# neobotix/neo_mpc_planner2

Measured on AMD Instinct MI355X. Metric: MPC solves/sec (control_steps=3, 500x500 costmap), higher is better.
Workload: dtype f64

## Files before the change

neo_mpc_planner2_amd/csrc/adjoint.h:

```cpp
#pragma once
#include "neo_mpc_device.h"
#include "wave_ops.h"
#include "fast_math.h"
#include "solver_context.h"
#include "costmap.h"
#include "riccati.h"

namespace neo_mpc {
namespace {

template <bool kTame, bool kRiccati, int kFew = 0>
__device__ __forceinline__ void adjoint_by_scans(const SolveArgs& a, const Ctx& c, double* L, bool exact_step, int lane, int n,
                                                 bool& free_path, int& nhops) {
  auto scan = [](double v) { if constexpr (kFew > 0) return wave_scan_few<kFew>(v); else return wave_scan(v); };
  constexpr int kLast = kFew > 0 ? kFew - 1 : 63;
  const DevParams& p = a.p;
  const double* u = L + a.lds.u;
  double* gs = L + a.lds.gs;
  float* RS = reinterpret_cast<float*>(L + a.lds.ric);
  float* ARTF = reinterpret_cast<float*>(L + a.lds.rt);
  const bool on = lane < n;
  const double vx = on ? u[3 * lane] : 0.0, vy = on ? u[3 * lane + 1] : 0.0, w = on ? u[3 * lane + 2] : 0.0;
  const double th = scan(w * p.dt);
  double sn, cs;
  sincos_heading<kTame>(th, &sn, &cs);
  const double ddx = (vx * cs - vy * sn) * p.dt, ddy = (vx * sn + vy * cs) * p.dt;
  const double x = scan(ddx), y = scan(ddy);
  double rt = on ? -2.0 * p.wo_n * (c.tyaw - th) : 0.0;
  if (lane == n - 1) rt += -2.0 * p.wterm_o * (c.fyaw - th);
  const double rx = on ? -2.0 * p.wt_n * (c.cx - x) : 0.0, ry = on ? -2.0 * p.wt_n * (c.cy - y) : 0.0;
  const double px = scan(rx), py = scan(ry);
  const double SX = lane_value(px, kLast) - px + rx, SY = lane_value(py, kLast) - py + ry;
  const double tt = on ? rt - ddy * SX + ddx * SY : 0.0;
  const double pt = scan(tt);
  const double ST = lane_value(pt, kLast) - pt + tt;
  int raw_here = 0;
  bool has_hop = false;
  float hop_x = 0.0f, hop_y = 0.0f;
  if (on) {
    gs[3 * lane] = p.dt * (cs * SX + sn * SY);
    gs[3 * lane + 1] = p.dt * (-sn * SX + cs * SY);
    gs[3 * lane + 2] = p.dt * ST;
    if (kRiccati) {
      float* rs = RS + kRicStage * lane;
      rs[RS_CS] = (float)cs; rs[RS_SN] = (float)sn; rs[RS_PX] = (float)ddx; rs[RS_PY] = (float)ddy;
      double wxx, wxy, wyy, wlx, wly;
      raw_here = edge_stickiness(a, c, L, x, y, cs, sn, wxx, wxy, wyy, wlx, wly, has_hop, hop_x, hop_y);
      rs[RS_WXX] = (float)wxx; rs[RS_WXY] = (float)wxy; rs[RS_WYY] = (float)wyy;
      rs[RS_WLX] = (float)wlx; rs[RS_WLY] = (float)wly;
      rs[RS_SY] = exact_step ? (float)SY : 0.0f;
      ARTF[2 * lane + 1] = exact_step ? (float)SX : 0.0f;
    }
  }
  if (kRiccati) {
    free_path = __ballot(raw_here != 0) == 0ull;
    const unsigned long long hmask = __ballot(has_hop);
    const int rank = __popcll(hmask & ((1ull << lane) - 1ull));
    double* t = L + a.lds.tol;
    if (has_hop && rank < kHopLanes) {
      reinterpret_cast<int*>(t + T_HOP_STAGE)[rank] = lane;
      reinterpret_cast<float*>(t + T_HOP_VEC)[2 * rank] = hop_x;
      reinterpret_cast<float*>(t + T_HOP_VEC)[2 * rank + 1] = hop_y;
    }
    nhops = min(__popcll(hmask), (int)kHopLanes);
    if (lane == 0) reinterpret_cast<int*>(t + T_HOP_STAGE)[kHopLanes] = nhops;
  }
  WAVE_SYNC();
}

template <int kSteps, bool kTame>
__device__ __forceinline__ void adjoint_short_sweep(const SolveArgs& a, const Ctx& c, double* L, bool have_trig, int lane, int n) {
  const DevParams& p = a.p;
  const double* u = L + a.lds.u;
  double* gs = L + a.lds.gs;
  double* ACS = L + a.lds.cs;
  double* ASN = L + a.lds.sn;
  double* ADX = L + a.lds.dxs;
  double* ADY = L + a.lds.dys;
  double* ARX = L + a.lds.rx;
  double* ARY = L + a.lds.ry;
  double* ART = L + a.lds.rt;
  double x = 0.0, y = 0.0, th = 0.0;
#pragma unroll
  for (int i = 0; i < n; ++i) {
    const double vx = u[3 * i], vy = u[3 * i + 1], w = u[3 * i + 2];
    th += w * p.dt;
    double sn, cs;
    if (kSteps && have_trig) { sn = ASN[i]; cs = ACS[i]; }
    else sincos_heading<kTame>(th, &sn, &cs);
    const double ddx = (vx * cs - vy * sn) * p.dt, ddy = (vx * sn + vy * cs) * p.dt;
    x += ddx; y += ddy;
    double rt = -2.0 * p.wo_n * (c.tyaw - th);
    if (i == n - 1) rt += -2.0 * p.wterm_o * (c.fyaw - th);
    if (lane == 0) {
      ACS[i] = cs; ASN[i] = sn; ADX[i] = ddx; ADY[i] = ddy;
      ARX[i] = -2.0 * p.wt_n * (c.cx - x); ARY[i] = -2.0 * p.wt_n * (c.cy - y); ART[i] = rt;
    }
  }
  WAVE_SYNC();
  double SX = 0.0, SY = 0.0, ST = 0.0;
#pragma unroll
  for (int k = n - 1; k >= 0; --k) {
    SX += ARX[k]; SY += ARY[k];
    ST += ART[k] - ADY[k] * SX + ADX[k] * SY;
    if (lane == 0) {
      gs[3 * k] = p.dt * (ACS[k] * SX + ASN[k] * SY);
      gs[3 * k + 1] = p.dt * (-ASN[k] * SX + ACS[k] * SY);
      gs[3 * k + 2] = p.dt * ST;
    }
  }
  WAVE_SYNC();
}

}
}
```

neo_mpc_planner2_amd/csrc/costmap.h:

```cpp
#pragma once
#include <hip/hip_runtime.h>
#include <math.h>
#include <stdint.h>

#include "neo_mpc_device.h"
#include "wave_ops.h"
#include "solver_context.h"
#include "fast_math.h"
#include "solver_rules.h"

namespace neo_mpc {
namespace {

__device__ __forceinline__ int cell_of(double w, double origin, double res, double inv) {
  double t = w - origin;
  double q = t * inv;
  double fl = floor(q);
  if (fabs(q - rint(q)) < 1e-6) fl = floor(t / res);
  int cell;
  asm("v_cvt_i32_f64 %0, %1" : "=v"(cell) : "v"(fl));
  return cell;
}

__device__ __forceinline__ int map_raw(const DevMap& m, int mx, int my) {
  if (mx < -m.border || my < -m.border || mx >= m.size_x + m.border || my >= m.size_y + m.border)
    return 254;
  return m.cells[(long)my * m.pitch + mx];
}

__device__ __forceinline__ int raw_occupancy(int raw) {
  return raw == 0 ? 0 : raw == 253 ? 99 : raw == 254 ? 100 : raw == 255 ? -1 : 1 + (97 * (raw - 1)) / 251;
}
__device__ __forceinline__ double raw_cost(int raw) { return (double)raw_occupancy(raw) / 100.0; }

template <bool kCovered = false>
__device__ __forceinline__ int cell_raw(const SolveArgs& a, const Ctx& c, const double* L, int mx, int my) {
  const unsigned tx = (unsigned)(mx - c.tile_x0), ty = (unsigned)(my - c.tile_y0);
  const int lg = c.tile_geom & 31;
  if (kCovered || ((tx >> lg) == 0u && ty < (unsigned)(c.tile_geom >> 8)))
    return reinterpret_cast<const uint8_t*>(L + a.lds.tile)[(ty << lg) + tx];
  return map_raw(a.map, mx, my);
}

template <bool kCovered = false>
__device__ __forceinline__ int step_raw(const SolveArgs& a, const Ctx& c, const double* L, double x, double y) {
  if (c.tile_geom & kTileFree) return 0;
  const double X = c.X0 + (c.c0 * x - c.s0 * y), Y = c.Y0 + (c.s0 * x + c.c0 * y);
  const int mx = cell_of(X, a.map.origin_x, a.map.resolution, a.map.inv_resolution);
  const int my = cell_of(Y, a.map.origin_y, a.map.resolution, a.map.inv_resolution);
  return cell_raw<kCovered>(a, c, L, mx, my);
}
template <bool kCovered = false>
__device__ __forceinline__ double step_term(const SolveArgs& a, const Ctx& c, const double* L, double x, double y) {
  return L[a.lds.term + step_raw<kCovered>(a, c, L, x, y)];
}

constexpr double kSticky = NEO_RULE_STICKY, kWall = NEO_RULE_WALL, kStickyDist = NEO_RULE_STICKY_DIST, kWallDist = NEO_RULE_WALL_DIST;
constexpr double kHopMargin = NEO_RULE_HOP_MARGIN;
template <bool kCovered = false>
__device__ __forceinline__ int edge_stickiness(const SolveArgs& a, const Ctx& c, const double* L, double x, double y,
                                               double cs, double sn, double& wxx, double& wxy, double& wyy, double& lx,
                                               double& ly, bool& hop, float& hop_x, float& hop_y) {
  wxx = 0.0; wxy = 0.0; wyy = 0.0; lx = 0.0; ly = 0.0;
  hop = false; hop_x = 0.0f; hop_y = 0.0f;
  if (c.tile_geom & kTileFree) return 0;
  double wt_n = a.p.wt_n;
  asm volatile("" : "+s"(wt_n));
  const double X = c.X0 + (c.c0 * x - c.s0 * y), Y = c.Y0 + (c.s0 * x + c.c0 * y);
  const int mx = cell_of(X, a.map.origin_x, a.map.resolution, a.map.inv_resolution);
  const int my = cell_of(Y, a.map.origin_y, a.map.resolution, a.map.inv_resolution);
  const double fx = (X - a.map.origin_x) * a.map.inv_resolution - (double)mx;
  const double fy = (Y - a.map.origin_y) * a.map.inv_resolution - (double)my;
  const int raw_here = cell_raw<kCovered>(a, c, L, mx, my);
  const double here = L[a.lds.term + raw_here];
  const bool far = mx <= -2147483647 || mx >= 2147483646 || my <= -2147483647 || my >= 2147483646;
  if (far) return raw_here;
  const double hop_range = L[a.lds.tol + T_HOP_RANGE];
  const double zone = fmax(kWallDist, hop_range);
  const bool xlo = fx < zone, xhi = 1.0 - fx < zone, ylo = fy < zone, yhi = 1.0 - fy < zone;
  double rx = 0.0, ry = 0.0, pbx = 0.0, pby = 0.0;
  double drop = L[a.lds.tol + T_HOP_DROP], hwx = 0.0, hwy = 0.0;
  if (xlo || xhi) {
    const int raw_n = cell_raw<kCovered>(a, c, L, xlo ? mx - 1 : mx + 1, my);
    const double dist = xlo ? fx : 1.0 - fx, there = L[a.lds.term + raw_n];
    const bool wall = raw_n == 254 && raw_here != 254;
    if (wall) { if (dist < kWallDist) { rx = kWall * 2.0 * wt_n; pbx = (xlo ? kWallDist - dist : dist - kWallDist) * a.map.resolution; } }
    else if (dist < kStickyDist && there > here) rx = kSticky * 2.0 * wt_n;
    if (dist < hop_range && here - there > drop) {
      drop = here - there; hop = true;
      hwx = (xlo ? -1.0 : 1.0) * (dist + kHopMargin) * a.map.resolution; hwy = 0.0;
    }
  }
  if (ylo || yhi) {
    const int raw_n = cell_raw<kCovered>(a, c, L, mx, ylo ? my - 1 : my + 1);
    const double dist = ylo ? fy : 1.0 - fy, there = L[a.lds.term + raw_n];
    const bool wall = raw_n == 254 && raw_here != 254;
    if (wall) { if (dist < kWallDist) { ry = kWall * 2.0 * wt_n; pby = (ylo ? kWallDist - dist : dist - kWallDist) * a.map.resolution; } }
    else if (dist < kStickyDist && there > here) ry = kSticky * 2.0 * wt_n;
    if (dist < hop_range && here - there > drop) {
      hop = true;
      hwx = 0.0; hwy = (ylo ? -1.0 : 1.0) * (dist + kHopMargin) * a.map.resolution;
    }
  }
  wxx = rx * c.c0 * c.c0 + ry * c.s0 * c.s0;
  wxy = rx * c.c0 * -c.s0 + ry * c.s0 * c.c0;
  wyy = rx * c.s0 * c.s0 + ry * c.c0 * c.c0;
  lx = -(rx * pbx * c.c0 + ry * pby * c.s0);
  ly = -(rx * pbx * -c.s0 + ry * pby * c.c0);
  if (hop) {
    const double hrx = c.c0 * hwx + c.s0 * hwy, hry = -c.s0 * hwx + c.c0 * hwy, idt = rcp_fast(a.p.dt);
    hop_x = (float)((cs * hrx + sn * hry) * idt); hop_y = (float)((-sn * hrx + cs * hry) * idt);
  }
  return raw_here;
}

__device__ double edge_cost(const DevMap& m, double ax, double ay, double bx, double by) {
  int x0 = cell_of(ax, m.origin_x, m.resolution, m.inv_resolution);
  int y0 = cell_of(ay, m.origin_y, m.resolution, m.inv_resolution);
  const int x1 = cell_of(bx, m.origin_x, m.resolution, m.inv_resolution);
  const int y1 = cell_of(by, m.origin_y, m.resolution, m.inv_resolution);
  if (x0 < 0 || y0 < 0 || x0 >= m.size_x || y0 >= m.size_y || x1 < 0 || y1 < 0 || x1 >= m.size_x || y1 >= m.size_y)
    return raw_cost(254);
  const long dx = labs((long)x1 - x0), dy = labs((long)y1 - y0);
  const int sx = x1 >= x0 ? 1 : -1, sy = y1 >= y0 ? 1 : -1;
  long err = dx - dy;
  double worst = -1.0;
  for (long guard = 0; guard <= dx + dy + 1; ++guard) {
    worst = fmax(worst, raw_cost(map_raw(m, x0, y0)));
    if (x0 == x1 && y0 == y1) break;
    long e2 = 2 * err;
    if (e2 > -dy) { err -= dy; x0 += sx; }
    if (e2 < dx) { err += dx; y0 += sy; }
  }
  return worst;
}

__device__ double footprint_cost(const SolveArgs& a, const double* L, uint32_t b, int lane) {
  if (!a.footprints || a.footprint_points == 0) return L[a.lds.prob + P_FOOTPRINT];
  const int np = (int)a.footprint_points;
  const double* pts = a.footprints + (size_t)b * 2 * np;
  double worst = -1.0;
  for (int e = lane; e < np; e += kLanes) {
    int j = (e + 1) % np;
    worst = fmax(worst, edge_cost(a.map, pts[2 * e], pts[2 * e + 1], pts[2 * j], pts[2 * j + 1]));
  }
  return wave_max(worst);
}

}
}
```

neo_mpc_planner2_amd/csrc/k1_solve.h:

```cpp
#pragma once
#include <hip/hip_runtime.h>
#include <hip/hip_ext.h>
#include <math.h>
#include <stdint.h>
#include <stdlib.h>

#include "neo_mpc_device.h"
#include "wave_ops.h"
#include "fast_math.h"
#include "solver_context.h"
#include "solver_rules.h"
#include "costmap.h"
#include "feasible_set.h"
#include "rollout.h"
#include "riccati.h"
#include "adjoint.h"
#include "tangent_cone.h"
#include "dense_newton.h"
#include "lbfgs.h"
#include "cell_scan.h"
#include "k1_timing.h"

namespace neo_mpc {
namespace {
// ... 75 lines not shown
    select_map(a.map, L + a.lds.prob);
    flags = reset_and_warm(a, L, b, lane) ? NEO_MPC_FLAG_RESET : 0;
    const double fcost = footprint_cost(a, L, b, lane);
    if (lane == 0) L[a.lds.prob + P_FOOTPRINT] = fcost;
    Ctx c;
    make_ctx_wave(p, a.map, L + a.lds.prob, fcost, c, lane);
    load_tile(a, c, L, lane);
    s.wall_in_reach = (c.tile_geom & kTileWall) != 0;
    if (s.wall_in_reach) flags |= NEO_MPC_FLAG_WALL_IN_REACH;
    if (lane == 0) {
      double* t = L + a.lds.tol;
      t[T_XTOL] = p.xtol; t[T_EARLY] = p.early_tol; t[T_FINAL] = p.final_tol; t[T_FTOL] = p.ftol;
      t[T_STALL] = p.stall_step; t[T_WTOL] = p.wtol; t[T_WTOL_LATE] = p.wtol_late; t[T_KINK] = p.kink_radius;
      t[T_KONST] = c.konst; t[T_TRUE_YAW] = c.true_yaw;
      t[T_HOP_DROP] = p.hop_min_drop; t[T_HOP_RANGE] = p.hop_range;
      t[T_BTOL_MAP] = p.btol_map; t[T_BTOL_FREE] = p.btol_free;
      reinterpret_cast<int*>(t + T_HOP_STAGE)[kHopLanes] = 0;
      t[T_C0] = c.c0; t[T_S0] = c.s0; t[T_TYAW] = c.tyaw; t[T_FYAW] = c.fyaw;
      int* ti = reinterpret_cast<int*>(t + T_TILE);
      ti[0] = c.tile_x0; ti[1] = c.tile_y0; ti[2] = c.tile_geom;
    }
    double* u = L + a.lds.u;
    for (int i = lane; i < n; i += kLanes) project_block<kTame>(p, u[3 * i], u[3 * i + 1], u[3 * i + 2]);
    WAVE_SYNC();
    for (int k = 0; k < nv; ++k) cold = cold && (u[k] == 0.0);
    ctx_from_lds<false>(a, L, c);
    {
      double* S = L + a.lds.state;
      int* Si = reinterpret_cast<int*>(S);
      const bool has_prev = uniform_int(Si[SI_HAS_PREV]) == 1 && !(flags & NEO_MPC_FLAG_RESET);
      WAVE_SYNC();
      if (lane == 0) {
        double q0 = has_prev ? S[S_PREV_U0] : u[nv - 3], q1 = has_prev ? S[S_PREV_U0 + 1] : u[nv - 2], q2 = has_prev ? S[S_PREV_U0 + 2] : u[nv - 1];
        project_block<kTame>(p, q0, q1, q2);
        S[S_PREV_U0] = q0; S[S_PREV_U0 + 1] = q1; S[S_PREV_U0 + 2] = q2;
        Si[SI_HAS_PREV] = 0;
      }
      WAVE_SYNC();
    }
    if (!cold && n > 1 && !(p.compat & kCompatNoUnshift) && p.max_it < kDumpGradient) {
      const double* A0 = L + a.lds.state + S_PREV_U0;
      double ts = 0.0;
      const double fs = rollout_cost<kSteps, kTame, kCovered>(
          a, c, L,
          [&](int i, double& b0, double& b1, double& b2) {
            const double* src = lane == 1 ? (i == 0 ? A0 : u + 3 * (i - 1)) : u + 3 * i;
            b0 = src[0]; b1 = src[1]; b2 = src[2];
          },
          NoRecord(), &ts);
      const double f_warm = lane_value(fs, 0), f_alt = lane_value(fs, 1);
      const bool free_both = lane_value(ts, 0) == 0.0 && lane_value(ts, 1) == 0.0;
      if (f_alt < f_warm && free_both) {
        double v0 = 0.0, v1 = 0.0, v2 = 0.0;
        const int k0 = lane, k1 = lane + kLanes, k2 = lane + 2 * kLanes;
        if (k0 < nv) v0 = k0 >= 3 ? u[k0 - 3] : A0[k0];
        if (k1 < nv) v1 = u[k1 - 3];
        if (k2 < nv) v2 = u[k2 - 3];
        WAVE_SYNC();
        if (k0 < nv) u[k0] = v0;
        if (k1 < nv) u[k1] = v1;
        if (k2 < nv) u[k2] = v2;
      } else if (f_alt < f_warm && lane == 0) {
        reinterpret_cast<int*>(L + a.lds.state)[SI_HAS_PREV] = kAltArmed;
      }
      WAVE_SYNC();
    }
  }
  s.flags = flags; s.cold = cold;
  return true;
}

template <int kMinWavesPerSimd, int kSteps, int kDir, bool kTame, int kStaticTile, int kLayoutSteps, bool kRouted = false>
__device__ __forceinline__ bool solve_search(double* L, uint32_t b, SolveCarry& sc) {
  constexpr bool kCovered = kStaticTile > 0;
  constexpr bool kNewton = kDir == 1;
  constexpr bool kRiccati = kDir == 2;
  constexpr bool kSecond = kDir != 0;
  constexpr bool kBlockedRule = kNewton || kRouted;
  static_assert(!kRiccati || kSteps == 0 || kRouted, "the stage-wise direction: run-time-sized, or the routed kernel's control_steps-3 branch");
  static_assert(!kRouted || (kRiccati && kSteps == kRoutedSteps), "the routed branch is the stage-wise one, three stages in registers");
  constexpr int kFew = (kRiccati && kSteps > 0) ? kSteps : 0;
  constexpr bool kHandOff = kFew > 0;
  constexpr bool kScalarCase = kFew > 0 && kTame;
  constexpr int kNwSteps = !kNewton ? 1 : kSteps ? kSteps : kNewtonMaxSteps;
  constexpr bool kVectorPose = kTame;
  constexpr int kRegSteps = kSteps ? kSteps : 1;
  constexpr int kPairs = kSteps ? 4 : NEO_MPC_MAX_LBFGS_MEMORY;
  double f = sc.f;
  const bool cold = sc.cold;
  int npairs = 0, head = 0, nfev = sc.nfev, it = sc.it, status = sc.status;
  neo_search_run run;
  neo_search_run_init(&run);
  double u_term = 0.0;
  double alpha = 1.0;
  bool scanned = false;
  int nscans = 0;
  bool scan_only = false;
  auto lane_again = []() {
    int zero;
    asm volatile("v_mov_b32 %0, 0" : "=v"(zero));
    return (int)__builtin_amdgcn_mbcnt_hi(~0u, __builtin_amdgcn_mbcnt_lo(~0u, (unsigned)zero));
  };
  NEO_SEGMENT_DECL;
  NEO_SEGMENT(0);
  for (;;) {
  SolveArgs a;
  fresh_args<kSteps, kStaticTile, kLayoutSteps, kRouted>(a);
  own_loop_params(a);
  select_map(a.map, L + a.lds.prob);
  const DevParams& p = a.p;
  const int n = kSteps ? kSteps : p.n, nv = 3 * n, mem = p.mem;
  double cand[3 * kRegSteps], cand_sn[kRegSteps], cand_cs[kRegSteps];
  bool have_trig = false;
  Ctx c;
  ctx_from_lds<kVectorPose>(a, L, c);
  double* u = L + a.lds.u;
  double* gs = L + a.lds.gs;
  double* gt = L + a.lds.gt;
  double* gr = L + a.lds.gr;
  double* d = L + a.lds.d;
  double* u_prev = L + a.lds.u_prev;
  double* gt_prev = L + a.lds.gt_prev;
  double* u_new = L + a.lds.u_new;
  double* ACS = L + a.lds.cs;
  double* ASN = L + a.lds.sn;
  int* AMODE = reinterpret_cast<int*>(L + a.lds.mode);
  static_assert(2 * 7 >= kNewtonRecord, "Newton records do not fit the step arrays");

  if (!scanned && nscans == 0) {
    const int lane = lane_again();
    for (int i = lane; i < n; i += kLanes) { AMODE[4 * i + 2] = 0; AMODE[4 * i + 3] = 0; }
    if (kRouted && lane == 0) L[a.lds.tol + T_KINK] = p.kink_radius_stagewise;
    alpha = kRiccati ? fmax(1.0, n * 0.125) : 1.0;
    if (kFew && lane == 0) { double* t = L + a.lds.tol; t[T_GAIN1] = INFINITY; t[T_GAIN2] = INFINITY; t[T_ALPHA] = alpha; }
    if (kRiccati && lane == 0) L[a.lds.tol + T_MU] = n > 8 ? (double)(n - 8) * 0.125 : 0.0;
  }
  bool v_feasible = false;
  if (kRiccati) {
    double b0 = c.v0, b1 = c.v1, b2 = c.v2;
    asm volatile("" : "+v"(b0), "+v"(b1), "+v"(b2));
    project_block<kTame>(p, b0, b1, b2);
    v_feasible = b0 == c.v0 && b1 == c.v1 && b2 == c.v2;
  }
  double my_scale;
  {
    int l0 = lane_again();
    my_scale = kRiccati ? 0.0 : lane_scale<kSecond>(l0);
  }
  for (; it < p.max_it && !scan_only; ++it) {
    int lane = lane_again();
    const bool exact_step = kRiccati && run.nblocked == 0;
    int tol_off = a.lds.tol;
    asm volatile("" : "+s"(tol_off));
    const double* TOL = L + tol_off;
    NEO_PHASE_DECL;
    NEO_PHASE(0);
    constexpr int kVars = 3 * kNwSteps;
    const int nvr = kSteps ? kVars : nv;
    bool free_path = false;
    int nhops = 0;
    float hc[kVars];
    float newton_sol = 0.0f;
    float dm_reg = 0.0f;
    int near_reg = 0;
    if (kNewton) {
      double hcol[kSteps ? kVars : 1];
      const double hstep = 1e-6, inv_h = 1.0 / hstep;
      double pcs[kNwSteps], psn[kNwSteps];
      double x = 0.0, y = 0.0, th = 0.0;
    #pragma unroll
      for (int i = 0; i < kNwSteps; ++i) {
        if (kSteps || i < n) {
          const double vx = u[3 * i] + (lane == 3 * i ? hstep : 0.0);
          const double vy = u[3 * i + 1] + (lane == 3 * i + 1 ? hstep : 0.0);
          const double w = u[3 * i + 2] + (lane == 3 * i + 2 ? hstep : 0.0);
          th += w * p.dt;
          sincos_heading<kTame>(th, &psn[i], &pcs[i]);
          x += (vx * pcs[i] - vy * psn[i]) * p.dt;
          y += (vx * psn[i] + vy * pcs[i]) * p.dt;
        }
      }
      double SX = 0.0, SY = 0.0, ST = 0.0;
    #pragma unroll
      for (int k = kNwSteps - 1; k >= 0; --k) {
        if (kSteps || k < n) {
          const double vx = u[3 * k] + (lane == 3 * k ? hstep : 0.0);
          const double vy = u[3 * k + 1] + (lane == 3 * k + 1 ? hstep : 0.0);
          const double w = u[3 * k + 2] + (lane == 3 * k + 2 ? hstep : 0.0);
          const double pdx = (vx * pcs[k] - vy * psn[k]) * p.dt, pdy = (vx * psn[k] + vy * pcs[k]) * p.dt;
          double prt = -2.0 * p.wo_n * (c.tyaw - th);
          if (k == n - 1) prt += -2.0 * p.wterm_o * (c.fyaw - th);
          SX += -2.0 * p.wt_n * (c.cx - x); SY += -2.0 * p.wt_n * (c.cy - y);
          ST += prt - pdy * SX + pdx * SY;
          const double g0 = p.dt * (pcs[k] * SX + psn[k] * SY), g1 = p.dt * (-psn[k] * SX + pcs[k] * SY),
                       g2 = p.dt * ST;
          if (kSteps) {
            hcol[3 * k] = g0; hcol[3 * k + 1] = g1; hcol[3 * k + 2] = g2;
          } else {
            const double b0 = lane_value(g0, 63), b1 = lane_value(g1, 63), b2 = lane_value(g2, 63);
            if (lane == 63) { gs[3 * k] = b0; gs[3 * k + 1] = b1; gs[3 * k + 2] = b2; }
            hc[3 * k] = (float)((g0 - b0) * inv_h);
            hc[3 * k + 1] = (float)((g1 - b1) * inv_h);
            hc[3 * k + 2] = (float)((g2 - b2) * inv_h);
          }
          x -= pdx; y -= pdy; th -= w * p.dt;
        } else {
          hc[3 * k] = 0.0f; hc[3 * k + 1] = 0.0f; hc[3 * k + 2] = 0.0f;
        }
      }
      if (kSteps) {
    #pragma unroll
        for (int j = 0; j < kVars; ++j) {
          const double base = lane_value(hcol[j], 63);
          if (lane == 63) gs[j] = base;
          hc[j] = (float)((hcol[j] - base) * inv_h);
        }
      }
      WAVE_SYNC();
    }
    else if (!kSteps || kRiccati) adjoint_by_scans<kTame, kRiccati, kFew>(a, c, L, exact_step, lane, n, free_path, nhops);
    else adjoint_short_sweep<kSteps, kTame>(a, c, L, have_trig, lane, n);
    NEO_PHASE(1);
    const bool my_corner = tangent_cone_pass<kTame, kNewton, kRiccati>(a, c, L, TOL[T_KINK], lane, n);
    WAVE_SYNC();
    const bool corner_any = kSecond && !kTame && __ballot(my_corner) != 0ull && (kRiccati ? free_path : (it > 0 && u_term == 0.0));
    NEO_PHASE(2);
    if (p.max_it == kDumpGradient) {
      for (int k = lane; k < nv; k += kLanes) a.solution[(size_t)b * nv + k] = gt[k];
      return true;
    }
    if (kSecond && it == 0 && cold) {
      if (kRiccati) { for (int k = lane; k < nv; k += kLanes) d[k] = -gr[k]; }
      else if (lane < nvr) d[lane] = -gr[lane];
      if (kRiccati) for (int i = lane; i < n; i += kLanes) AMODE[4 * i + 3] = 0;
      WAVE_SYNC();
    } else if (kRiccati) {
      const int my_flags = riccati_prepare(a, c, L, n, lane, v_feasible, (float)TOL[T_MU]);
      int stage_flags[kFew ? kFew : 1] = {};
      if (kScalarCase) {
        for (int i = 0; i < kFew; ++i) stage_flags[i] = __builtin_amdgcn_readlane(my_flags, i);
      }
      WAVE_SYNC();
      if (corner_any) riccati_keep_linear_terms(a, L, n, lane, true);
      auto sweep = [&]() {
        SweepHandOff<float> ho = {};
        riccati_sweep<float, (kMinWavesPerSimd < 4), kFew, kHandOff, kScalarCase>(a, L, n, lane, &ho, stage_flags);
        riccati_finish<kHandOff>(a, c, L, n, lane, &ho, &dm_reg);
        near_reg = ho.near;
      };
      sweep();
      if (!kTame && corner_any && repin_corner_blocks<true>(a, L, n, lane)) {
        riccati_keep_linear_terms(a, L, n, lane, false);
        sweep();
      }
    } else if (kNewton) {
      newton_sol = dense_newton_direction<kSteps, kNwSteps, kTame>(a, L, hc, corner_any, lane, n, nvr);
    }
    NEO_PHASE(3);
    if (!kSecond) lbfgs_direction<kSteps, kPairs>(a, L, it, mem, head, npairs, lane, n);
    if (kSecond && it > 0) {
      float dm = 0.0f;
      int anynear = 0;
      if (kHandOff) {
        dm = dm_reg;
        anynear = near_reg == 1;
      } else if (kRiccati) {
        for (int k = lane; k < nv; k += kLanes) {
          const float v = (float)fabs(d[k]);
          dm = (v == v) ? fmaxf(dm, v) : INFINITY;
          anynear |= (AMODE[4 * (k / 3) + 2] == 1);
        }
      } else if (lane < nvr) { dm = fabsf(newton_sol); anynear = (AMODE[4 * (lane / 3) + 2] == 1); }
      if constexpr (kHandOff) dm = wave_max_f_few<kFew>(dm);
      else if constexpr (kFew > 0 && 3 * kFew <= 16) dm = wave_max_f_few<3 * kFew>(dm); else dm = wave_max_f(dm);
      const bool near_any = __ballot(anynear != 0) != 0ull;
      const int verdict = neo_rules_step_test((double)dm, near_any, nhops, TOL[T_EARLY], TOL[T_FINAL], kRiccati && !exact_step);
      if (verdict == NEO_STEP_CONVERGED) { status = NEO_MPC_STATUS_CONVERGED; break; }
      if (verdict == NEO_STEP_IS_LAST) run.final_step = true;
    }
    NEO_PHASE(4);
    if (p.max_it > kDumpGradient && it == p.max_it - kDumpGradient - 1) {
      for (int k = lane; k < nv; k += kLanes) a.solution[(size_t)b * nv + k] = d[k];
      return true;
    }
    const double lscale = kRiccati ? lane_scale<kSecond>(lane) : my_scale;
    const double alpha_now = kFew ? TOL[T_ALPHA] : alpha;
    const double pstep = alpha_now * lscale;
    const double step = lane < 32 ? pstep : lscale;
    bool took_trial = false;
    double fb = INFINITY, cterm = 0.0;
    int best = 32;
    if (kRiccati && free_path && it > 0) took_trial = riccati_free_space_trial<kTame, kCovered, kFew, kBlockedRule>(a, c, L, n, lane, alpha_now, f, fb, cterm);
    const double* ALT0 = L + a.lds.state + S_PREV_U0;
    bool alt_armed = false;
    if (it == 0) alt_armed = uniform_int(reinterpret_cast<const int*>(L + a.lds.state)[SI_HAS_PREV]) == kAltArmed;
    if (!took_trial) {
    int hop_stage = -1;
    float hop_x = 0.0f, hop_y = 0.0f;
    if (kRiccati && lane >= 1 && lane <= nhops) {
      const double* t = TOL;
      hop_stage = reinterpret_cast<const int*>(t + T_HOP_STAGE)[lane - 1];
      hop_x = reinterpret_cast<const float*>(t + T_HOP_VEC)[2 * (lane - 1)];
      hop_y = reinterpret_cast<const float*>(t + T_HOP_VEC)[2 * (lane - 1) + 1];
    }
    double fc = rollout_cost<kSteps, kTame, kCovered>(
        a, c, L,
        [&](int i, double& b0, double& b1, double& b2) {
          candidate_block<kTame, kRiccati, (kFew > 0 && kTame)>(a, c, L, lane, step, pstep, i, b0, b1, b2, hop_stage, hop_x, hop_y);
          if (it == 0) {
            asm volatile("");
            if (lane == 0) { b0 = u[3 * i]; b1 = u[3 * i + 1]; b2 = u[3 * i + 2]; }
            if (lane == kAltLane && alt_armed) { const double* src = i == 0 ? ALT0 : u + 3 * (i - 1); b0 = src[0]; b1 = src[1]; b2 = src[2]; }
          }
          if (kSteps) { cand[3 * i] = b0; cand[3 * i + 1] = b1; cand[3 * i + 2] = b2; }
        },
        [&](int i, double sn, double cs) {
          if (kSteps && !kSecond) { cand_sn[i] = sn; cand_cs[i] = cs; }
        }, kBlockedRule ? &cterm : nullptr);
    NEO_PHASE(5);
    if (!(fc == fc)) fc = INFINITY;
    if (it == 0) { f = lane_value(fc, 0); if (kNewton) u_term = lane_value(cterm, 0); }
    fb = fc;
    best = lane;
    wave_argmin(fb, best);
    }
    ++nfev;
    if (!(fb < f)) { status = NEO_MPC_STATUS_CONVERGED; ++it; break; }
    const bool alt_won = alt_armed && best == kAltLane;
    float stepmax = 0.0f;
    if (kSteps && kSecond && !took_trial) {
      if (lane == best) {
#pragma unroll
        for (int k = 0; k < 3 * kRegSteps; ++k) {
          stepmax = fmaxf(stepmax, (float)fabs(cand[k] - u[k]));
          u[k] = cand[k];
        }
      }
      stepmax = __builtin_bit_cast(float, __builtin_amdgcn_readlane(__builtin_bit_cast(int, stepmax), best));
      have_trig = true;
    } else {
      if (kSteps && !kSecond) {
        if (lane == best) {
#pragma unroll
          for (int i = 0; i < kRegSteps; ++i) {
            u_new[3 * i] = cand[3 * i]; u_new[3 * i + 1] = cand[3 * i + 1]; u_new[3 * i + 2] = cand[3 * i + 2];
            ASN[i] = cand_sn[i]; ACS[i] = cand_cs[i];
          }
        }
      } else if (!kSteps && !took_trial) {
        const double bstep = lane_value(step, best), bpstep = lane_value(pstep, best);
        int bhop = -1;
        float bhx = 0.0f, bhy = 0.0f;
        if (kRiccati && best >= 1 && best <= nhops) {
          bhop = reinterpret_cast<const int*>(TOL + T_HOP_STAGE)[best - 1];
          bhx = reinterpret_cast<const float*>(TOL + T_HOP_VEC)[2 * (best - 1)];
          bhy = reinterpret_cast<const float*>(TOL + T_HOP_VEC)[2 * (best - 1) + 1];
        }
        for (int i = lane; i < n; i += kLanes) {
          double b0, b1, b2;
          candidate_block<kTame, kRiccati>(a, c, L, best, bstep, bpstep, i, b0, b1, b2, bhop, bhx, bhy);
          if (alt_won) { const double* src = i == 0 ? ALT0 : u + 3 * (i - 1); b0 = src[0]; b1 = src[1]; b2 = src[2]; }
          u_new[3 * i] = b0; u_new[3 * i + 1] = b1; u_new[3 * i + 2] = b2;
        }
      }
      have_trig = true;
      WAVE_SYNC();
      for (int k = lane; k < nv; k += kLanes) {
        const double nu = u_new[k], ou = u[k];
        stepmax = fmaxf(stepmax, (float)fabs(nu - ou));
        if (!kSecond) { u_prev[k] = ou; gt_prev[k] = gt[k]; }
        u[k] = nu;
      }
      stepmax = wave_max_f(stepmax);
    }
    const bool hop_won = (kRiccati && best >= 1 && best <= nhops) || alt_won;
    const bool free_rollout = kBlockedRule ? lane_value(cterm, best) == 0.0 : false;
    const bool free_now = kRiccati ? free_path : (kNewton ? free_rollout : false);
    if (kFew) { run.gain1 = TOL[T_GAIN1]; run.gain2 = TOL[T_GAIN2]; }
    const double gain = kNewton ? lane_value(f - fb, 0) : f - fb;
    const bool ends = neo_rules_iteration_ends(kRiccati, kRouted, kBlockedRule, TOL, &run, it, best >= 32, lane_value(step, best), hop_won,
                                               gain, fb, (double)stepmax, free_now, free_rollout);
    double* TOLW = L + tol_off;
    if (kFew) { if (lane == 0) { TOLW[T_GAIN2] = run.gain2; TOLW[T_GAIN1] = run.gain1; } }
    f = fb;
    if (kNewton) u_term = lane_value(cterm, best);
    if (kRiccati && !(it == 0 && cold) && !hop_won) {
      constexpr unsigned long long kNearlyFull = newton_lanes_at_least(NEO_RULE_DAMP_RELAX_STEP),
                                   kShort = kNewtonLanes & ~newton_lanes_at_least(NEO_RULE_DAMP_TIGHTEN_STEP);
      const double mu0 = n > 8 ? (double)(n - 8) * 0.125 : 0.0, mu = TOL[T_MU];
      double* mu_slot = L + tol_off + T_MU;
      if ((kNearlyFull >> best) & 1ull) { if (lane == 0) *mu_slot = fmax(NEO_RULE_DAMP_RELAX * mu, mu0 * (1.0 / NEO_RULE_DAMP_RANGE)); }
      else if (best < 32 || ((kShort >> best) & 1ull)) { if (lane == 0) *mu_slot = fmin(NEO_RULE_DAMP_TIGHTEN * mu, NEO_RULE_DAMP_RANGE * mu0); }
    }
    if (best < 32 && !hop_won) {
      const double al = clampd(lane_value(step, best), 1e-6, 1e6);
      if (kFew) { if (lane == 0) TOLW[T_ALPHA] = al; }
      else alpha = al;
    }
    WAVE_SYNC();
    NEO_PHASE(6);
    NEO_PHASE_DUMP();
    if (ends) { status = NEO_MPC_STATUS_CONVERGED; ++it; break; }
  }

  if (!kSecond || scanned || status != NEO_MPC_STATUS_CONVERGED || p.max_it >= kDumpGradient) break;
  const bool nothing_to_scan = (c.tile_geom & kTileFree) || (kNewton && u_term == 0.0);
  if (nothing_to_scan && nscans == 0) break;
  bool resume = false;
  {
    SolveArgs as;
    fresh_args<kSteps, kStaticTile, kLayoutSteps, kRouted>(as);
    select_map(as.map, L + as.lds.prob);
    Ctx cs;
    ctx_from_lds<false>(as, L, cs);
    int ls = lane_again();
    if (nscans == 0 && ls == 0) L[as.lds.tol + T_FSCAN] = f;
    NEO_SEGMENT_SCAN_BEGIN();
    const bool w = !nothing_to_scan &&
                   cell_scan<kSteps, kTame, kCovered>(as, cs, L, f, kNewton ? &u_term : nullptr, nfev, ls, kSteps ? kSteps : as.p.n);
    NEO_SEGMENT_SCAN_END();
    ++nscans;
    scan_only = w && nscans < NEO_RULE_SCAN_REPEATS;
    if (!scan_only) {
      scanned = true;
      WAVE_SYNC();
      resume = L[as.lds.tol + T_FSCAN] - f > as.p.scan_resume_gain && it < as.p.max_it;
      if (kFew && resume) {
        if (ls == 0) { L[as.lds.tol + T_GAIN1] = INFINITY; L[as.lds.tol + T_GAIN2] = INFINITY; }
        WAVE_SYNC();
      }
    }
  }
  if (scan_only) continue;
  if (!resume) break;
  status = NEO_MPC_STATUS_MAX_ITER;
  neo_search_run_init(&run);
  }
  NEO_SEGMENT(1);
  NEO_SEGMENT_DUMP();
  if (scanned && status == NEO_MPC_STATUS_MAX_ITER) status = NEO_MPC_STATUS_CONVERGED;
  sc.f = f; sc.it = it; sc.nfev = nfev; sc.status = status;
  return false;
}

template <int kSteps, int kStaticTile, int kLayoutSteps>
__device__ __forceinline__ void solve_finish(double* L, uint32_t b, int lane, const SolveCarry& sc) {
  const int flags = sc.flags, status = sc.status, it = sc.it, nfev = sc.nfev;
  double f = sc.f;
  SolveArgs a;
  fresh_args<kSteps, kStaticTile, kLayoutSteps>(a);
  select_map(a.map, L + a.lds.prob);
  const DevParams& p = a.p;
  const int n = kSteps ? kSteps : p.n, nv = 3 * n;
  double* u = L + a.lds.u;
  Ctx c;
  ctx_from_lds<false>(a, L, c);
#ifndef NEO_MPC_PHASE_TIMING
  if (a.solution && p.max_it < kDumpGradient)
    for (int k = lane; k < nv; k += kLanes) a.solution[(size_t)b * nv + k] = u[k];
#endif
  WAVE_SYNC();
  f += L[a.lds.tol + T_KONST];
  c.true_yaw = L[a.lds.tol + T_TRUE_YAW];
// ... 63 lines not shown
```

neo_mpc_planner2_amd/csrc/solver_context.h:

```cpp
#pragma once
#include <hip/hip_runtime.h>
#include <math.h>
#include <stdint.h>

#include "neo_mpc_device.h"
#include "solver_rules.h"

namespace neo_mpc {
namespace {

enum : int {
  P_CUR_X = 0, P_CUR_Y = 1, P_CUR_Q = 2, P_CARROT_X = 6, P_CARROT_Y = 7, P_CARROT_Q = 8,
  P_GOAL = 12, P_GOAL_Q = 15, P_VEL = 19, P_INTERVAL = 22, P_DELTA_T = 23, P_FOOTPRINT = 24,
  PI_MAP_INDEX = 50,
  PI_SKIP = 52,
  kProblemDoubles = 27,
  kStateDoubles = 16,
  S_LAST = 0, S_OLD_GOAL = 3, S_WAIT = 10, SI_HAS_GOAL = 22, SI_COLLISION = 23, SI_COLL_FP = 24,
  SI_HAS_PREV = 25, S_PREV_U0 = 13, kAltArmed = 2, kAltLane = 5
};

enum : int { T_XTOL = NEO_TOL_XTOL, T_EARLY = NEO_TOL_EARLY, T_FINAL = NEO_TOL_FINAL, T_FTOL = NEO_TOL_FTOL, T_STALL = NEO_TOL_STALL,
             T_WTOL = NEO_TOL_WTOL, T_WTOL_LATE = NEO_TOL_WTOL_LATE, T_BTOL_MAP = NEO_TOL_BTOL_MAP, T_BTOL_FREE = NEO_TOL_BTOL_FREE,
             T_KINK = NEO_TOL_COUNT, T_KONST, T_TRUE_YAW, T_MU,
             T_HOP_STAGE = 13 , T_HOP_VEC = 16 , T_HOP_DROP = 20, T_HOP_RANGE = 21,
             T_C0 = 22, T_S0 = 23, T_TYAW = 24, T_FYAW = 25, T_TILE = 26 ,
             T_GAIN1 = 28, T_GAIN2 = 29, T_ALPHA = 30,
             T_FSCAN = 31 ,
             kTolDoubles = 32, kHopLanes = 4  };
static_assert(T_MU < T_HOP_STAGE, "the stop tolerances and the cold constants end in front of the hop table");

constexpr int kTileFree = 0x80;
constexpr int kTileWall = 0x40;

struct Ctx {
  double cx, cy, tyaw, fyaw, c0, s0, X0, Y0, v0, v1, v2, konst, true_yaw;
  int tile_x0, tile_y0;
  int tile_geom;
};

}
}
```

neo_mpc_planner2_amd/csrc/tangent_cone.h:

```cpp
#pragma once
#include "neo_mpc_device.h"
#include "fast_math.h"
#include "solver_context.h"
#include "solver_rules.h"
#include "riccati.h"

namespace neo_mpc {
namespace {

constexpr int kNewtonRecord = 13;

template <bool kTame, bool kNewton, bool kRiccati>
__device__ __forceinline__ bool tangent_cone_pass(const SolveArgs& a, const Ctx& c, double* L, double kink_radius, int lane, int n) {
  constexpr bool kSecond = kNewton || kRiccati;
  const DevParams& p = a.p;
  const double* u = L + a.lds.u;
  double* gs = L + a.lds.gs;
  double* gt = L + a.lds.gt;
  double* gr = L + a.lds.gr;
  double* ANX = L + a.lds.nx;
  double* ANY = L + a.lds.ny;
  int* AMODE = reinterpret_cast<int*>(L + a.lds.mode);
  float* NB = reinterpret_cast<float*>(L + a.lds.cs);
  float* ARTF = reinterpret_cast<float*>(L + a.lds.rt);
  bool my_corner = false;
  for (int i = lane; i < n; i += kLanes) {
    const double u0 = u[3 * i], u1 = u[3 * i + 1], u2 = u[3 * i + 2];
    const double g0 = gs[3 * i], g1 = gs[3 * i + 1], g2 = gs[3 * i + 2];
    const double e0 = u0 - c.v0, e1 = u1 - c.v1, e2 = u2 - c.v2;
    const double ne2 = e0 * e0 + e1 * e1 + e2 * e2;
    const double ine = ne2 > 0.0 ? rsq_fast(ne2) : 0.0;
    const double ne = ne2 * ine;
    double t0, t1, t2;
    if (ne2 > 0.0) {
      const double wn = p.wc_n * ine;
      t0 = g0 + wn * e0; t1 = g1 + wn * e1; t2 = g2 + wn * e2;
    } else {
      const double ng2 = g0 * g0 + g1 * g1 + g2 * g2;
      const double sh = (ng2 > p.wc_n * p.wc_n) ? 1.0 - p.wc_n * rsq_fast(ng2) : 0.0;
      t0 = g0 * sh; t1 = g1 * sh; t2 = g2 * sh;
    }
    if (!kRiccati) AMODE[4 * i + 3] = AMODE[4 * i + 2];
    const bool near = ne < kink_radius;
    if (near) { t0 = g0; t1 = g1; t2 = g2; }
    else { gt[3 * i] = t0; gt[3 * i + 1] = t1; gt[3 * i + 2] = t2; }
    const int wfroz = ((u2 <= p.lo[2] && t2 > 0.0) || (u2 >= p.hi[2] && t2 < 0.0)) ? 1 : 0;
    double r0 = t0, r1 = t1;
    double nx0 = 0.0, ny0 = 0.0, nx1 = 0.0, ny1 = 0.0, nx2 = 0.0, ny2 = 0.0;
    bool v0 = false, v1 = false, v2 = false;
    if (!kTame && !p.disc_in_box) {
      constexpr double kRoom = NEO_RULE_CORNER_ROOM;
      if (u0 <= p.lo[0] + kRoom) { nx0 = -1.0; v0 = true; }
      else if (u0 >= p.hi[0] - kRoom) { nx0 = 1.0; v0 = true; }
      if (u1 <= p.lo[1] + kRoom) { ny1 = -1.0; v1 = true; }
      else if (u1 >= p.hi[1] - kRoom) { ny1 = 1.0; v1 = true; }
    }
    const double nvv2 = u0 * u0 + u1 * u1, rlim = p.r * (1.0 - 1e-12);
    if (nvv2 > 0.0 && nvv2 >= rlim * rlim) { const double iv = rsq_fast(nvv2); nx2 = u0 * iv; ny2 = u1 * iv; v2 = true; }
    const double dx = -t0, dy = -t1;
    const double dn0 = nx0 * dx + ny0 * dy, dn1 = nx1 * dx + ny1 * dy, dn2 = nx2 * dx + ny2 * dy;
    int mode = 0, mslot = -1;
    double mnx = 0.0, mny = 0.0, mlam = 0.0;
    if ((v0 && dn0 > 0.0) || (v1 && dn1 > 0.0) || (v2 && dn2 > 0.0)) {
      double bestn = -1.0;
      mode = 2;
#define NEO_TRY_SLIDE(sk, vk, dnk, nxk, nyk, va, nxa, nya, vb, nxb, nyb)                               \
      if (vk && dnk > 0.0) {                                                                         \
        const double px = dx - dnk * nxk, py = dy - dnk * nyk;                                       \
        const double tol = 1e-14 * (fabs(px) + fabs(py));                                            \
        const bool ok = !(va && nxa * px + nya * py > tol) && !(vb && nxb * px + nyb * py > tol);    \
        const double pn = px * px + py * py;                                                         \
        if (ok && pn > bestn) {                                                                      \
          bestn = pn; mode = 1; mnx = nxk; mny = nyk; r0 = -px; r1 = -py; mslot = sk; mlam = dnk;     \
        }                                                                                            \
      }
      NEO_TRY_SLIDE(2, v2, dn2, nx2, ny2, v0, nx0, ny0, v1, nx1, ny1)
      NEO_TRY_SLIDE(0, v0, dn0, nx0, ny0, v1, nx1, ny1, v2, nx2, ny2)
      NEO_TRY_SLIDE(1, v1, dn1, nx1, ny1, v0, nx0, ny0, v2, nx2, ny2)
#undef NEO_TRY_SLIDE
      if (mode == 2) { r0 = 0.0; r1 = 0.0; }
    }
    if (near) {
      const double s2 = wfroz ? 0.0 : t2;
      gs[3 * i] = r0; gs[3 * i + 1] = r1; gs[3 * i + 2] = s2;
      gt[3 * i] = 0.0; gt[3 * i + 1] = 0.0; gt[3 * i + 2] = 0.0;
      gr[3 * i] = 0.0; gr[3 * i + 1] = 0.0; gr[3 * i + 2] = 0.0;
      const int at_rest = (ne2 == 0.0 && r0 * r0 + r1 * r1 + s2 * s2 <= p.wc_n * p.wc_n) ? 2 : 1;
      ANX[i] = 0.0; ANY[i] = 0.0; AMODE[4 * i] = 0; AMODE[4 * i + 1] = 0; AMODE[4 * i + 2] = at_rest;
      if (kNewton) {
#pragma unroll
        for (int k = 0; k < kNewtonRecord; ++k) NB[kNewtonRecord * i + k] = 0.0f;
      }
      if (kRiccati) ARTF[2 * i] = 0.0f;
      continue;
    }
    gr[3 * i] = r0; gr[3 * i + 1] = r1; gr[3 * i + 2] = wfroz ? 0.0 : t2;
    if (kSecond && !kTame && !p.disc_in_box && mode == 1) {
      const double room = NEO_RULE_CORNER_ROOM, rin = p.r - room;
      my_corner = my_corner || (mslot != 0 && (u0 - p.lo[0] <= room || p.hi[0] - u0 <= room)) ||
                  (mslot != 1 && (u1 - p.lo[1] <= room || p.hi[1] - u1 <= room)) || (mslot != 2 && nvv2 >= rin * rin);
    }
    ANX[i] = mnx; ANY[i] = mny; AMODE[4 * i] = mode; AMODE[4 * i + 1] = wfroz | ((mode == 1 && mslot == 2) ? 2 : 0); AMODE[4 * i + 2] = 0;
    if (kNewton) {
      float* nb = NB + kNewtonRecord * i;
      nb[0] = mode == 0 ? 1.0f : mode == 1 ? (float)(1.0 - mnx * mnx) : 0.0f;
      nb[1] = mode == 1 ? (float)(-mnx * mny) : 0.0f;
      nb[2] = mode == 0 ? 1.0f : mode == 1 ? (float)(1.0 - mny * mny) : 0.0f;
      nb[3] = wfroz ? 0.0f : 1.0f;
      const float f0 = (float)e0, f1 = (float)e1, f2 = (float)e2;
      const float fn2 = f0 * f0 + f1 * f1 + f2 * f2;
      const float ine = fn2 > 0.0f ? __builtin_amdgcn_rsqf(fn2) : 0.0f;
// ... 55 lines not shown
```

Measured before the change: 27.23 million.

## Carry stage values in registers, batch covered tile lookups, read tolerances from kernarg

The adjoint scan now hands each lane's controls and gradients to the tangent-cone pass in registers, so that pass no longer re-reads them from LDS. When the tile is known to cover the stage, the edge-stickiness check issues the here and neighbour tile and term lookups together up front instead of bounds-checked loads inside branches. The acceptance test reads its tolerance constants straight from the kernel-argument segment rather than from the LDS tolerance block. All of this is aimed at cutting LDS latency on the short-horizon tame Riccati path, in exchange for more register pressure and speculative neighbour loads that may go unused.

```diff
diff --git a/neo_mpc_planner2_amd/csrc/adjoint.h b/neo_mpc_planner2_amd/csrc/adjoint.h
--- a/neo_mpc_planner2_amd/csrc/adjoint.h
+++ b/neo_mpc_planner2_amd/csrc/adjoint.h
@@ -9,9 +9,9 @@
 namespace neo_mpc {
 namespace {
 
-template <bool kTame, bool kRiccati, int kFew = 0>
+template <bool kTame, bool kRiccati, int kFew = 0, bool kCovered = false>
 __device__ __forceinline__ void adjoint_by_scans(const SolveArgs& a, const Ctx& c, double* L, bool exact_step, int lane, int n,
-                                                 bool& free_path, int& nhops) {
+                                                 bool& free_path, int& nhops, StageCarry* carry = nullptr) {
   auto scan = [](double v) { if constexpr (kFew > 0) return wave_scan_few<kFew>(v); else return wave_scan(v); };
   constexpr int kLast = kFew > 0 ? kFew - 1 : 63;
   const DevParams& p = a.p;
@@ -45,11 +45,17 @@
       float* rs = RS + kRicStage * lane;
       rs[RS_CS] = (float)cs; rs[RS_SN] = (float)sn; rs[RS_PX] = (float)ddx; rs[RS_PY] = (float)ddy;
       double wxx, wxy, wyy, wlx, wly;
-      raw_here = edge_stickiness(a, c, L, x, y, cs, sn, wxx, wxy, wyy, wlx, wly, has_hop, hop_x, hop_y);
+      raw_here = edge_stickiness<kCovered>(a, c, L, x, y, cs, sn, wxx, wxy, wyy, wlx, wly, has_hop, hop_x, hop_y);
       rs[RS_WXX] = (float)wxx; rs[RS_WXY] = (float)wxy; rs[RS_WYY] = (float)wyy;
       rs[RS_WLX] = (float)wlx; rs[RS_WLY] = (float)wly;
       rs[RS_SY] = exact_step ? (float)SY : 0.0f;
       ARTF[2 * lane + 1] = exact_step ? (float)SX : 0.0f;
+    }
+    if (kFew > 0 && carry) {
+      int off = 3 * lane;
+      asm volatile("" : "+v"(off));
+      carry->u0 = u[off]; carry->u1 = u[off + 1]; carry->u2 = u[off + 2];
+      carry->g0 = gs[off]; carry->g1 = gs[off + 1]; carry->g2 = gs[off + 2];
     }
   }
   if (kRiccati) {
diff --git a/neo_mpc_planner2_amd/csrc/costmap.h b/neo_mpc_planner2_amd/csrc/costmap.h
--- a/neo_mpc_planner2_amd/csrc/costmap.h
+++ b/neo_mpc_planner2_amd/csrc/costmap.h
@@ -71,18 +71,35 @@
   const int my = cell_of(Y, a.map.origin_y, a.map.resolution, a.map.inv_resolution);
   const double fx = (X - a.map.origin_x) * a.map.inv_resolution - (double)mx;
   const double fy = (Y - a.map.origin_y) * a.map.inv_resolution - (double)my;
-  const int raw_here = cell_raw<kCovered>(a, c, L, mx, my);
-  const double here = L[a.lds.term + raw_here];
+  double hop_range, drop;
+  if (kCovered) { hop_range = L[a.lds.tol + T_HOP_RANGE]; drop = L[a.lds.tol + T_HOP_DROP]; }
+  int raw_here, raw_nx = 0, raw_ny = 0;
+  double here, there_x = 0.0, there_y = 0.0;
+  if (kCovered) {
+    const double zone0 = fmax(kWallDist, hop_range);
+    const unsigned tx = (unsigned)mx - (unsigned)c.tile_x0, ty = (unsigned)my - (unsigned)c.tile_y0;
+    const unsigned ntx = fx < zone0 ? tx - 1u : tx + 1u, nty = fy < zone0 ? ty - 1u : ty + 1u;
+    const int lg = c.tile_geom & 31;
+    const uint8_t* tile = reinterpret_cast<const uint8_t*>(L + a.lds.tile);
+    raw_here = tile[(ty << lg) + tx]; raw_nx = tile[(ty << lg) + ntx]; raw_ny = tile[(nty << lg) + tx];
+    asm volatile("" : "+v"(raw_here), "+v"(raw_nx), "+v"(raw_ny));
+    here = L[a.lds.term + raw_here]; there_x = L[a.lds.term + raw_nx]; there_y = L[a.lds.term + raw_ny];
+    asm volatile("" : "+v"(here), "+v"(there_x), "+v"(there_y));
+  } else {
+    raw_here = cell_raw<false>(a, c, L, mx, my);
+    here = L[a.lds.term + raw_here];
+  }
   const bool far = mx <= -2147483647 || mx >= 2147483646 || my <= -2147483647 || my >= 2147483646;
   if (far) return raw_here;
-  const double hop_range = L[a.lds.tol + T_HOP_RANGE];
+  if (!kCovered) hop_range = L[a.lds.tol + T_HOP_RANGE];
   const double zone = fmax(kWallDist, hop_range);
   const bool xlo = fx < zone, xhi = 1.0 - fx < zone, ylo = fy < zone, yhi = 1.0 - fy < zone;
   double rx = 0.0, ry = 0.0, pbx = 0.0, pby = 0.0;
-  double drop = L[a.lds.tol + T_HOP_DROP], hwx = 0.0, hwy = 0.0;
+  if (!kCovered) drop = L[a.lds.tol + T_HOP_DROP];
+  double hwx = 0.0, hwy = 0.0;
   if (xlo || xhi) {
-    const int raw_n = cell_raw<kCovered>(a, c, L, xlo ? mx - 1 : mx + 1, my);
-    const double dist = xlo ? fx : 1.0 - fx, there = L[a.lds.term + raw_n];
+    const int raw_n = kCovered ? raw_nx : cell_raw<false>(a, c, L, xlo ? mx - 1 : mx + 1, my);
+    const double dist = xlo ? fx : 1.0 - fx, there = kCovered ? there_x : L[a.lds.term + raw_n];
     const bool wall = raw_n == 254 && raw_here != 254;
     if (wall) { if (dist < kWallDist) { rx = kWall * 2.0 * wt_n; pbx = (xlo ? kWallDist - dist : dist - kWallDist) * a.map.resolution; } }
     else if (dist < kStickyDist && there > here) rx = kSticky * 2.0 * wt_n;
@@ -92,8 +109,8 @@
     }
   }
   if (ylo || yhi) {
-    const int raw_n = cell_raw<kCovered>(a, c, L, mx, ylo ? my - 1 : my + 1);
-    const double dist = ylo ? fy : 1.0 - fy, there = L[a.lds.term + raw_n];
+    const int raw_n = kCovered ? raw_ny : cell_raw<false>(a, c, L, mx, ylo ? my - 1 : my + 1);
+    const double dist = ylo ? fy : 1.0 - fy, there = kCovered ? there_y : L[a.lds.term + raw_n];
     const bool wall = raw_n == 254 && raw_here != 254;
     if (wall) { if (dist < kWallDist) { ry = kWall * 2.0 * wt_n; pby = (ylo ? kWallDist - dist : dist - kWallDist) * a.map.resolution; } }
     else if (dist < kStickyDist && there > here) ry = kSticky * 2.0 * wt_n;
diff --git a/neo_mpc_planner2_amd/csrc/k1_solve.h b/neo_mpc_planner2_amd/csrc/k1_solve.h
--- a/neo_mpc_planner2_amd/csrc/k1_solve.h
+++ b/neo_mpc_planner2_amd/csrc/k1_solve.h
@@ -181,6 +181,8 @@
   constexpr int kFew = (kRiccati && kSteps > 0) ? kSteps : 0;
   constexpr bool kHandOff = kFew > 0;
   constexpr bool kScalarCase = kFew > 0 && kTame;
+  constexpr bool kStageCarry = kFew > 0 && kTame;
+  constexpr bool kAcceptFetch = kFew > 0 && kTame;
   constexpr int kNwSteps = !kNewton ? 1 : kSteps ? kSteps : kNewtonMaxSteps;
   constexpr bool kVectorPose = kTame;
   constexpr int kRegSteps = kSteps ? kSteps : 1;
@@ -262,6 +264,7 @@
     float newton_sol = 0.0f;
     float dm_reg = 0.0f;
     int near_reg = 0;
+    StageCarry carry = {};
     if (kNewton) {
       double hcol[kSteps ? kVars : 1];
       const double hstep = 1e-6, inv_h = 1.0 / hstep;
@@ -317,10 +320,10 @@
       }
       WAVE_SYNC();
     }
-    else if (!kSteps || kRiccati) adjoint_by_scans<kTame, kRiccati, kFew>(a, c, L, exact_step, lane, n, free_path, nhops);
+    else if (!kSteps || kRiccati) adjoint_by_scans<kTame, kRiccati, kFew, kCovered>(a, c, L, exact_step, lane, n, free_path, nhops, kStageCarry ? &carry : nullptr);
     else adjoint_short_sweep<kSteps, kTame>(a, c, L, have_trig, lane, n);
     NEO_PHASE(1);
-    const bool my_corner = tangent_cone_pass<kTame, kNewton, kRiccati>(a, c, L, TOL[T_KINK], lane, n);
+    const bool my_corner = tangent_cone_pass<kTame, kNewton, kRiccati>(a, c, L, TOL[T_KINK], lane, n, kStageCarry ? &carry : nullptr);
     WAVE_SYNC();
     const bool corner_any = kSecond && !kTame && __ballot(my_corner) != 0ull && (kRiccati ? free_path : (it > 0 && u_term == 0.0));
     NEO_PHASE(2);
@@ -475,9 +478,17 @@
     const bool hop_won = (kRiccati && best >= 1 && best <= nhops) || alt_won;
     const bool free_rollout = kBlockedRule ? lane_value(cterm, best) == 0.0 : false;
     const bool free_now = kRiccati ? free_path : (kNewton ? free_rollout : false);
+    double tolk[NEO_TOL_COUNT] = {};
+    if (kAcceptFetch) {
+      auto kp = (const __attribute__((address_space(4))) char*)__builtin_amdgcn_kernarg_segment_ptr();
+      asm volatile("" : "+s"(kp));
+      const DevParams& q = ((const SolveArgs*)kp)->p;
+      tolk[NEO_TOL_XTOL] = q.xtol; tolk[NEO_TOL_FTOL] = q.ftol; tolk[NEO_TOL_STALL] = q.stall_step; tolk[NEO_TOL_WTOL] = q.wtol;
+      tolk[NEO_TOL_WTOL_LATE] = q.wtol_late; tolk[NEO_TOL_BTOL_MAP] = q.btol_map; tolk[NEO_TOL_BTOL_FREE] = q.btol_free;
+    }
     if (kFew) { run.gain1 = TOL[T_GAIN1]; run.gain2 = TOL[T_GAIN2]; }
     const double gain = kNewton ? lane_value(f - fb, 0) : f - fb;
-    const bool ends = neo_rules_iteration_ends(kRiccati, kRouted, kBlockedRule, TOL, &run, it, best >= 32, lane_value(step, best), hop_won,
+    const bool ends = neo_rules_iteration_ends(kRiccati, kRouted, kBlockedRule, kAcceptFetch ? tolk : TOL, &run, it, best >= 32, lane_value(step, best), hop_won,
                                                gain, fb, (double)stepmax, free_now, free_rollout);
     double* TOLW = L + tol_off;
     if (kFew) { if (lane == 0) { TOLW[T_GAIN2] = run.gain2; TOLW[T_GAIN1] = run.gain1; } }
diff --git a/neo_mpc_planner2_amd/csrc/solver_context.h b/neo_mpc_planner2_amd/csrc/solver_context.h
--- a/neo_mpc_planner2_amd/csrc/solver_context.h
+++ b/neo_mpc_planner2_amd/csrc/solver_context.h
@@ -39,5 +39,7 @@
   int tile_geom;
 };
 
+struct StageCarry { double u0, u1, u2, g0, g1, g2; };
+
 }
 }
diff --git a/neo_mpc_planner2_amd/csrc/tangent_cone.h b/neo_mpc_planner2_amd/csrc/tangent_cone.h
--- a/neo_mpc_planner2_amd/csrc/tangent_cone.h
+++ b/neo_mpc_planner2_amd/csrc/tangent_cone.h
@@ -11,7 +11,8 @@
 constexpr int kNewtonRecord = 13;
 
 template <bool kTame, bool kNewton, bool kRiccati>
-__device__ __forceinline__ bool tangent_cone_pass(const SolveArgs& a, const Ctx& c, double* L, double kink_radius, int lane, int n) {
+__device__ __forceinline__ bool tangent_cone_pass(const SolveArgs& a, const Ctx& c, double* L, double kink_radius, int lane, int n,
+                                                  const StageCarry* carry = nullptr) {
   constexpr bool kSecond = kNewton || kRiccati;
   const DevParams& p = a.p;
   const double* u = L + a.lds.u;
@@ -25,8 +26,13 @@
   float* ARTF = reinterpret_cast<float*>(L + a.lds.rt);
   bool my_corner = false;
   for (int i = lane; i < n; i += kLanes) {
-    const double u0 = u[3 * i], u1 = u[3 * i + 1], u2 = u[3 * i + 2];
-    const double g0 = gs[3 * i], g1 = gs[3 * i + 1], g2 = gs[3 * i + 2];
+    double u0, u1, u2, g0, g1, g2;
+    if (carry) {
+      u0 = carry->u0; u1 = carry->u1; u2 = carry->u2; g0 = carry->g0; g1 = carry->g1; g2 = carry->g2;
+    } else {
+      u0 = u[3 * i]; u1 = u[3 * i + 1]; u2 = u[3 * i + 2];
+      g0 = gs[3 * i]; g1 = gs[3 * i + 1]; g2 = gs[3 * i + 2];
+    }
     const double e0 = u0 - c.v0, e1 = u1 - c.v1, e2 = u2 - c.v2;
     const double ne2 = e0 * e0 + e1 * e1 + e2 * e2;
     const double ine = ne2 > 0.0 ? rsq_fast(ne2) : 0.0;
```

After: 28.09 million (median of 6 runs). 1.03x the previous value.
